# codyheiser/MILWRM

Measured on AMD Instinct MI355X. Metric: pixels/sec (node) for preprocess+k-means fit+label, 30-ch MxIF k=8; %HBM peak, higher is better.
Workload: dtype f32 (fp64 accumulation)

## Files before the change

include/milwrm_amd.h:

```cpp
#ifndef MILWRM_AMD_H
#define MILWRM_AMD_H

#include <stddef.h>
#include <stdint.h>

#ifdef __cplusplus
extern "C" {
#endif

#define MW_OK 0
#define MW_EINVAL (-1)
#define MW_EHIP (-2)
#define MW_EUNSUPPORTED (-3)

#define MW_U8 0
#define MW_U16 1
#define MW_F32 2

int mw_version(void);
const char* mw_last_error(void);
int mw_stream_blocks(int64_t n);
int64_t mw_rows_per_block(int64_t n);

size_t mw_nz_stats_ws_bytes(int64_t n_pix, int C);
// ... 234 lines not shown
  int64_t msg_len;
  int (*all_reduce_sum)(void* ctx, int64_t off, int64_t n, void* stream);
  int (*all_gather)(void* ctx, int64_t in_off, int64_t n, int64_t out_off, void* stream);
} mw_fit_comm;
int64_t mw_lloyd_fits_msg_len(int64_t rec_total, int F, int world);
int mw_lloyd_fits_sharded(const float* d_X, int64_t S, int F, const float* d_a32, const float* d_b32,
                          const int32_t* d_qexp, const float* h_a32, const float* h_b32,
                          const int32_t* h_qexp, const float* h_xmax, const double* h_mu,
                          const double* h_inv, int n, const int* h_k, const double* h_init,
                          uint8_t* const* d_labels, float* const* d_ub, float* const* d_lb,
                          void* const* d_ws, float* d_par, double* d_out, int max_iter, double tol,
                          int first_kind, int queue_kind, double queue_below, int dense_min,
                          int nobound, double* h_centers, double* h_inertia, int* h_n_iter,
                          int64_t* h_hist, int hist_cap, int* h_hist_len, double* h_timing,
                          const mw_fit_comm* comm, void* stream);

size_t mw_farthest_ws_bytes(int64_t S);
int mw_farthest(const float* d_X, int64_t S, int F, const float* d_a,
                const float* d_b, const double* d_centers, int k,
                const uint8_t* d_labels, int n, int64_t* d_top_idx,
                double* d_top_val, void* d_ws, void* stream);

size_t mw_assign_ws_bytes(int64_t n_pix, int k);
int mw_assign_conf(const float* d_img, int C, const int32_t* d_feat, int F,
                   const float* d_a, const float* d_b, const float* d_centers,
                   int k, const uint8_t* d_mask, int64_t n_pix,
                   int8_t* d_label, float* d_conf, void* d_ws, void* stream);
int mw_blur_assign_conf(const void* d_img, int dtype, int H, int W, int C, const float* d_inv_mean,
                        float pseudoval, const float* h_weights, int radius, const float* d_a,
                        const float* d_b, const float* d_centers, int k, const uint8_t* d_mask,
// ... 40 lines not shown
```

milwrm_amd/_native.py:

```python
from __future__ import annotations

import ctypes as C
import os
import threading

import torch

_HERE = os.path.dirname(os.path.abspath(__file__))
LIB_PATH = os.environ.get("MW_LIB") or os.path.join(_HERE, "libmilwrm_amd.so")

MW_U8, MW_U16, MW_F32 = 0, 1, 2
_EINVAL, _EHIP, _EUNSUP = -1, -2, -3

_lib = None
_lock = threading.Lock()

c_i64, c_i32, c_u32, c_u64 = C.c_int64, C.c_int, C.c_uint32, C.c_uint64
c_f32, c_sz, c_vp = C.c_float, C.c_size_t, C.c_void_p
c_dp = C.POINTER(C.c_double)

_PROTOS = {
    "mw_version": (c_i32, []),
    "mw_host_labels_f64": (c_i32, [c_vp, c_i64, c_vp, c_i32]),
    "mw_host_f32_to_f64": (c_i32, [c_vp, c_i64, c_vp, c_i32]),
# ... 75 lines not shown
                                            c_vp, c_vp]),
    "mw_kmeans_fit_deferred": (c_i32, [c_vp, c_i64, c_i32, c_vp, c_vp, c_vp, c_vp, c_i32, c_vp, c_u32, c_i32,
                                       C.c_double, c_vp, c_vp, c_vp, c_vp, c_vp, c_sz, c_i32, c_vp, c_vp, c_vp]),
    "mw_kmeans_fit_finish_ws_bytes": (c_sz, [c_i64, c_i32, c_i32]),
    "mw_kmeans_fit_finish": (c_i32, [c_vp, c_i64, c_i32, c_vp, c_vp, c_vp, c_i32, c_vp, c_i32, c_vp, c_vp, c_sz,
                                     c_vp, c_vp, c_vp]),
    "mw_lloyd_fits": (c_i32, [c_vp, c_i64, c_i32, c_vp, c_vp, c_vp, c_vp, c_vp, c_vp, c_vp, c_vp, c_vp,
                              c_i32, c_vp, c_vp, c_vp, c_vp, c_vp, c_vp, c_vp, c_vp, c_i32, C.c_double,
                              c_i32, c_i32, C.c_double, c_i32, c_i32, c_vp, c_vp, c_vp, c_vp, c_i32, c_vp,
                              c_vp, c_vp]),
    "mw_lloyd_fits_msg_len": (c_i64, [c_i64, c_i32, c_i32]),
    "mw_lloyd_fits_sharded": (c_i32, [c_vp, c_i64, c_i32, c_vp, c_vp, c_vp, c_vp, c_vp, c_vp, c_vp, c_vp, c_vp,
                                      c_i32, c_vp, c_vp, c_vp, c_vp, c_vp, c_vp, c_vp, c_vp, c_i32, C.c_double,
                                      c_i32, c_i32, C.c_double, c_i32, c_i32, c_vp, c_vp, c_vp, c_vp, c_i32,
                                      c_vp, c_vp, c_vp, c_vp]),
    "mw_farthest_ws_bytes": (c_sz, [c_i64]),
    "mw_farthest": (c_i32, [c_vp, c_i64, c_i32, c_vp, c_vp, c_vp, c_i32, c_vp, c_i32, c_vp, c_vp, c_vp, c_vp]),
    "mw_assign_ws_bytes": (c_sz, [c_i64, c_i32]),
    "mw_assign_conf": (c_i32, [c_vp, c_i32, c_vp, c_i32, c_vp, c_vp, c_vp, c_i32, c_vp, c_i64, c_vp, c_vp, c_vp, c_vp]),
    "mw_assign_reduce": (c_i32, [c_vp, c_i64, c_i32, c_vp, c_vp]),
    "mw_domain_sse_ws_bytes": (c_sz, [c_i64, c_i32, c_i32]),
    "mw_domain_sse_out_len": (c_i32, [c_i32, c_i32]),
    "mw_domain_sse": (c_i32, [c_vp, c_i32, c_vp, c_i32, c_vp, c_vp, c_vp, c_vp, c_vp, c_i32, c_i32, c_vp,
                              c_i64, c_vp, c_i32, c_vp, c_vp]),
    "mw_domain_sse_f64": (c_i32, [c_vp, c_i32, c_vp, c_i32, c_vp, c_vp, c_vp, c_vp, c_vp, c_i32, c_i32, c_vp,
                                  c_i64, c_vp, c_i32, c_vp, c_vp]),
    "mw_neighbor_mean": (c_i32, [c_vp, c_vp, c_i64, c_vp, c_i32, c_vp, c_vp]),
    "mw_col_stats_rows": (c_i32, [c_vp, c_i64, c_i32, c_vp, c_vp]),
    "mw_col_stats_absmax": (c_i32, [c_vp, c_i64, c_i32, c_vp, c_i32, c_vp]),
    "mw_sample_slot_elems": (c_sz, [c_i64]),
# ... 100 lines not shown
```

milwrm_amd/csrc/fit.cpp:

```cpp
#include <hip/hip_runtime.h>

#include <algorithm>
#include <chrono>
#include <cmath>
#include <cstring>
#include <limits>
#include <vector>

#include "common.h"

#pragma clang fp contract(off)

namespace mw {
void mt_init_genrand(uint32_t seed, uint32_t* mt);
void mt_regen(uint32_t* mt);
int kpp_step(const float* d_X, int64_t S, int F, const double* d_mu, const double* d_inv, int c,
             const double* h_u, int T, void* d_ws, void* stream, bool store_cur);

namespace {

struct LegacyRandom {
  uint32_t mt[624];
  int pos = 624;
  explicit LegacyRandom(uint32_t seed) { mt_init_genrand(seed, mt); }
// ... 285 lines not shown
    for (int i = 0; i < n; ++i)
      MW_HIP(hipMemcpyAsync(r.data() + (size_t)i * F, X + idx[i] * F, F * sizeof(float),
                            hipMemcpyDeviceToHost, st));
    MW_HIP(hipStreamSynchronize(st));
    for (int i = 0; i < n; ++i)
      for (int f = 0; f < F; ++f)
        outv[(size_t)i * F + f] = ((double)r[(size_t)i * F + f] - mu[f]) * inv[f];
    return MW_OK;
  }
};

struct FitLayout {
  size_t small, par, ub, lb, lws, out, big, fold, total;
};
static inline size_t fal(size_t x) { return (x + 255) & ~(size_t)255; }
static int lloyd_queue_kind() {
  static const int q = [] {
    const char* e = getenv("MW_LLOYD_LIST");
    return (e && e[0] == '0') ? 2 : 4;
  }();
  return q;
}
static FitLayout fit_layout(int64_t S, int F, int k) {
  const int T = 2 + (int)std::log((double)(k < 1 ? 1 : k));
  FitLayout L;
  L.small = 0;
  L.par = fal(64 * 4 * 4 + 64 * 8 * 2 + 64 * 64 * 8 + 64 * 8 * 2 + 130 * 8 + 64 * 8);
  L.ub = L.par + fal(((size_t)k * F + 2 * k) * 4);
  L.lb = L.ub + fal((size_t)S * 4);
  L.lws = L.lb + fal((size_t)S * 4);
// ... 348 lines not shown
      if (h_init_idx) std::memcpy(h_init_idx, idx.data(), k * sizeof(int64_t));
    } else {
      MW_HIP(hipMemcpyAsync(idx.data(), d_idx, k * 8, hipMemcpyDeviceToHost, st));
      MW_HIP(hipStreamSynchronize(st));
      idx[0] = first;
      MW_TRY(fit.scaled_rows(idx.data(), k, h_mu, h_inv, centers));
      if (h_init_idx) std::memcpy(h_init_idx, idx.data(), k * sizeof(int64_t));
    }
  }

  fit_hist.clear();
  if (!fold) MW_HIP(hipMemsetAsync(d_labels, 255, (size_t)S, st));
  std::vector<int64_t> q_hi((size_t)k * F, 0), q_lo((size_t)k * F, 0), count(k, 0);
  std::vector<double> rec, cnew((size_t)k * F), weight(k), tmp(std::max(F, k));
  int64_t last_recomputed = -1;
  int n_iter = 0;
  bool done = false, strict = false;
  for (int it = 0; it < max_iter && !done; ++it) {
    MW_TRY(fit.upload(centers));
    static const int first_kind = [] {
      const char* e = getenv("MW_LLOYD_FIRST_ATOMIC");
      return (e && e[0] == '1') ? 3 : 0;
    }();
    static const double queue_below = [] {
      const char* e = getenv("MW_LLOYD_QUEUE_BELOW");
      return e ? atof(e) : 0.3;
    }();
    const int queue_kind = lloyd_queue_kind();
    int kind = first_kind;
    if (last_recomputed >= 0) {
      double frac = (double)last_recomputed / (double)S;
      if (fit.prev_dmax > 0.f && std::isfinite(fit.drift_max))
        frac *= std::min(1.0, (double)fit.drift_max / (double)fit.prev_dmax);
      kind = frac > queue_below ? 1 : queue_kind;
    }
    if (fold && it == 0) {
      MW_TRY(mw_lloyd_list_moved(d_moved, mw_kpp_best_ptr(big, S, T), S, F, k, fit.ws, st));
      MW_TRY(fit.pass(0, 8, 0, rec, true));
    } else {
      MW_TRY(fit.pass(0, kind, 0, rec));
    }
    for (size_t i = 0; i < (size_t)k * F; ++i) {
      q_hi[i] += (int64_t)rec[i];
      q_lo[i] += (int64_t)rec[(size_t)k * F + i];
      const int64_t carry = q_lo[i] >> 32;
      q_hi[i] += carry;
      q_lo[i] -= carry << 32;
    }
    for (int j = 0; j < k; ++j) count[j] += (int64_t)rec[2 * (size_t)k * F + j];
    const double* tail = rec.data() + 2 * (size_t)k * F + k;
    const int64_t changed = (int64_t)tail[0];
    last_recomputed = (int64_t)tail[1];
    fit_hist.insert(fit_hist.end(), {(int64_t)(fold && it == 0 ? 8 : kind), changed, last_recomputed,
                                     (int64_t)(tail[2] * 4294967296.0 + tail[3])});
    for (int j = 0; j < k; ++j) {
      weight[j] = (double)count[j];
      for (int f = 0; f < F; ++f) {
        const size_t i = (size_t)j * F + f;
        const double sx = ((double)q_hi[i] * 4294967296.0 + (double)q_lo[i]) * qscale[f];
        cnew[i] = fit.a64[f] * sx + fit.b64[f] * weight[j];
      }
    }
    std::vector<int> empty;
    for (int j = 0; j < k; ++j)
      if (weight[j] == 0.0) empty.push_back(j);
    if (!empty.empty()) {
      const int ne = (int)empty.size();
// ... 57 lines not shown

  *h_n_iter = n_iter;
  std::memcpy(h_centers, centers.data(), centers.size() * sizeof(double));
  if (h_strict) {
    *h_strict = strict ? 1 : 0;
    return MW_OK;
  }
  fit_hist.insert(fit_hist.end(), {(int64_t)(strict ? 12 : 11), -1, -1, S});
  return fit_tail(fit, xmax.data(), centers, strict, !own.p, h_inertia, h_final_rec, h_inertia_exp);
}

namespace mw {
namespace {

constexpr int kFitsMaxPerLaunch = 24;
constexpr int kKindFirst = 0, kKindTile = 1, kKindDense = 5;

struct FitsFit {
  int k = 0;
  std::vector<double> centers;
  std::vector<float> prev32;
  bool have_prev = false;
  std::vector<int64_t> q_hi, q_lo, count;
  bool done = false, strict = false, bounds_ok = true;
  int n_iter = 0;
  double drift_max = 0.0, prev_dmax = 0.0;
  int iexp = 0;
  std::vector<int64_t> hist;
};

void fits_tables(FitsFit& fs, int F, bool nobound, float* h) {
  const int k = fs.k;
  for (size_t i = 0; i < (size_t)k * F; ++i) h[i] = (float)fs.centers[i];
  const float inf = std::numeric_limits<float>::infinity();
  std::vector<float> drift32(k), half32(k);
  double dmax;
  if (nobound) {
    for (int j = 0; j < k; ++j) drift32[j] = inf, half32[j] = 0.f;
    dmax = std::numeric_limits<double>::infinity();
  } else {
    std::vector<double> tmp(F);
// ... 62 lines not shown
  ~TimedLaunches() {
    for (T& t : v) {
      (void)hipEventDestroy(t.a);
      (void)hipEventDestroy(t.b);
    }
  }
};

int lloyd_fits_impl(const float* d_X, int64_t S, int F, const float* d_a32, const float* d_b32,
                    const int32_t* d_qexp, const float* h_a32, const float* h_b32, const int32_t* h_qexp,
                    const float* h_xmax, const double* h_mu, const double* h_inv, int n, const int* h_k,
                    const double* h_init, uint8_t* const* d_labels, float* const* d_ub, float* const* d_lb,
                    void* const* d_ws, float* d_par, double* d_out, int max_iter, double tol, int first_kind,
                    int queue_kind, double queue_below, int dense_min, int nobound, double* h_centers,
                    double* h_inertia, int* h_n_iter, int64_t* h_hist, int hist_cap, int* h_hist_len,
                    double* h_timing, const mw_fit_comm* comm, void* stream);

}
}

extern "C" int mw_lloyd_fits(const float* d_X, int64_t S, int F, const float* d_a32, const float* d_b32,
                             const int32_t* d_qexp, const float* h_a32, const float* h_b32,
                             const int32_t* h_qexp, const float* h_xmax, const double* h_mu,
                             const double* h_inv, int n, const int* h_k, const double* h_init,
                             uint8_t* const* d_labels, float* const* d_ub, float* const* d_lb,
                             void* const* d_ws, float* d_par, double* d_out, int max_iter, double tol,
                             int first_kind, int queue_kind, double queue_below, int dense_min,
                             int nobound, double* h_centers, double* h_inertia, int* h_n_iter,
                             int64_t* h_hist, int hist_cap, int* h_hist_len, double* h_timing,
                             void* stream) {
  return lloyd_fits_impl(d_X, S, F, d_a32, d_b32, d_qexp, h_a32, h_b32, h_qexp, h_xmax, h_mu, h_inv, n, h_k,
                         h_init, d_labels, d_ub, d_lb, d_ws, d_par, d_out, max_iter, tol, first_kind, queue_kind,
                         queue_below, dense_min, nobound, h_centers, h_inertia, h_n_iter, h_hist, hist_cap,
                         h_hist_len, h_timing, nullptr, stream);
}

extern "C" int64_t mw_lloyd_fits_msg_len(int64_t rec_total, int F, int world) {
  if (rec_total < 0 || F < 1 || F > 64 || world < 1) return 0;
  return msg_layout(rec_total, F, world).total;
}

extern "C" int mw_lloyd_fits_sharded(const float* d_X, int64_t S, int F, const float* d_a32,
                                     const float* d_b32, const int32_t* d_qexp, const float* h_a32,
                                     const float* h_b32, const int32_t* h_qexp, const float* h_xmax,
                                     const double* h_mu, const double* h_inv, int n, const int* h_k,
                                     const double* h_init, uint8_t* const* d_labels, float* const* d_ub,
                                     float* const* d_lb, void* const* d_ws, float* d_par, double* d_out,
                                     int max_iter, double tol, int first_kind, int queue_kind,
                                     double queue_below, int dense_min, int nobound, double* h_centers,
                                     double* h_inertia, int* h_n_iter, int64_t* h_hist, int hist_cap,
                                     int* h_hist_len, double* h_timing, const mw_fit_comm* comm,
                                     void* stream) {
  MW_CHECK_ARG(comm && comm->d_msg && comm->all_reduce_sum && comm->all_gather,
               "mw_lloyd_fits_sharded: null comm");
  MW_CHECK_ARG(comm->world >= 1 && comm->rank >= 0 && comm->rank < comm->world && comm->row_offset >= 0 &&
                   comm->rows_total >= S + comm->row_offset,
               "mw_lloyd_fits_sharded: bad world / rank / row range");
  MW_CHECK_ARG(d_out == comm->d_msg, "mw_lloyd_fits_sharded: d_out must be comm->d_msg (records at offset 0)");
  return lloyd_fits_impl(d_X, S, F, d_a32, d_b32, d_qexp, h_a32, h_b32, h_qexp, h_xmax, h_mu, h_inv, n, h_k,
                         h_init, d_labels, d_ub, d_lb, d_ws, d_par, d_out, max_iter, tol, first_kind, queue_kind,
                         queue_below, dense_min, nobound, h_centers, h_inertia, h_n_iter, h_hist, hist_cap,
                         h_hist_len, h_timing, comm, stream);
}

namespace mw {
namespace {

int lloyd_fits_impl(const float* d_X, int64_t S, int F, const float* d_a32, const float* d_b32,
                    const int32_t* d_qexp, const float* h_a32, const float* h_b32, const int32_t* h_qexp,
                    const float* h_xmax, const double* h_mu, const double* h_inv, int n, const int* h_k,
                    const double* h_init, uint8_t* const* d_labels, float* const* d_ub, float* const* d_lb,
                    void* const* d_ws, float* d_par, double* d_out, int max_iter, double tol, int first_kind,
                    int queue_kind, double queue_below, int dense_min, int nobound, double* h_centers,
                    double* h_inertia, int* h_n_iter, int64_t* h_hist, int hist_cap, int* h_hist_len,
                    double* h_timing, const mw_fit_comm* comm, void* stream) {
  MW_CHECK_ARG(d_X && d_a32 && d_b32 && d_qexp && h_a32 && h_b32 && h_qexp && h_xmax && h_mu && h_inv &&
                   h_k && h_init && d_labels && d_ub && d_lb && d_ws && d_par && d_out && h_centers &&
                   h_inertia && h_n_iter,
               "mw_lloyd_fits: null pointer");
  MW_CHECK_ARG(n >= 1 && F >= 1 && F <= 64 && S >= 1 && max_iter >= 1 && tol >= 0.0,
               "mw_lloyd_fits: bad n / F / S / max_iter / tol");
  hipStream_t st = as_stream(stream);
  const int64_t S_glob = comm ? comm->rows_total : S;
  std::vector<FitsFit> fits(n);
  std::vector<int64_t> poff(n + 1, 0), roff(n + 1, 0);
  size_t coff = 0;
  for (int g = 0; g < n; ++g) {
    const int k = h_k[g];
    MW_CHECK_ARG(k >= 1 && k <= 64 && S >= k, "mw_lloyd_fits: fit %d: k=%d", g, k);
    FitsFit& fs = fits[g];
    fs.k = k;
    fs.centers.assign(h_init + coff, h_init + coff + (size_t)k * F);
    coff += (size_t)k * F;
    fs.q_hi.assign((size_t)k * F, 0);
    fs.q_lo.assign((size_t)k * F, 0);
    fs.count.assign(k, 0);
// ... 125 lines not shown
  double* d_c64 = nullptr;
  int64_t* d_topi = nullptr;
  double* d_topv = nullptr;
  void* d_farws = nullptr;

  int rc = MW_OK;
  std::vector<double> cnew, weight, tmp(std::max(F, kmax));
  for (int it = 0; it < max_iter && rc == MW_OK; ++it) {
    std::vector<int> active;
    for (int g = 0; g < n; ++g)
      if (!fits[g].done) active.push_back(g);
    if (active.empty()) break;
    const bool dense_now = dense_ok && it > 0 && (int)active.size() >= dense_min;
    if ((rc = upload(active)) != MW_OK) break;
    std::vector<int> by_kind[8];
    for (int g : active) {
      const FitsFit& fs = fits[g];
      int kind;
      if (fs.hist.empty()) {
        kind = first_kind;
      } else if (dense_now) {
        kind = kKindDense;
      } else if (!fs.bounds_ok) {
        kind = kKindTile;
      } else {
        double frac = (double)fs.hist.back() / (double)std::max<int64_t>(S_glob, 1);
        if (fs.prev_dmax > 0 && std::isfinite(fs.drift_max)) frac *= std::min(1.0, fs.drift_max / fs.prev_dmax);
        kind = frac > queue_below ? kKindTile : queue_kind;
      }
      by_kind[kind].push_back(g);
    }
    host_mark();
    for (int kind = 0; kind < 8 && rc == MW_OK; ++kind)
      if (!by_kind[kind].empty()) rc = launch(by_kind[kind], 0, kind);
    if (rc != MW_OK || (rc = download()) != MW_OK) break;
    for (int g : active) {
      FitsFit& fs = fits[g];
      const int k = fs.k;
      if (it > 0) fs.bounds_ok = !dense_now;
      const double* r = rec + roff[g];
      for (size_t i = 0; i < (size_t)k * F; ++i) {
        fs.q_hi[i] += (int64_t)r[i];
        fs.q_lo[i] += (int64_t)r[(size_t)k * F + i];
        const int64_t carry = fs.q_lo[i] >> 32;
        fs.q_hi[i] += carry;
        fs.q_lo[i] -= carry << 32;
      }
      for (int j = 0; j < k; ++j) fs.count[j] += (int64_t)r[2 * (size_t)k * F + j];
      const double* tail = r + 2 * (size_t)k * F + k;
      const int64_t changed = (int64_t)tail[0];
      fs.hist.push_back(changed);
      fs.hist.push_back((int64_t)tail[1]);
      cnew.assign((size_t)k * F, 0.0);
      weight.assign(k, 0.0);
      for (int j = 0; j < k; ++j) {
        weight[j] = (double)fs.count[j];
        for (int f = 0; f < F; ++f) {
          const size_t i = (size_t)j * F + f;
          const double sx = ((double)fs.q_hi[i] * 4294967296.0 + (double)fs.q_lo[i]) * qscale[f];
          cnew[i] = a64[f] * sx + b64[f] * weight[j];
        }
      }
      std::vector<int> empty;
      for (int j = 0; j < k; ++j)
        if (weight[j] == 0.0) empty.push_back(j);
      if (!empty.empty()) {
        const int ne = (int)empty.size();
// ... 198 lines not shown
```

milwrm_amd/csrc/lloyd.hip:

```cpp
#include <math.h>
#include <stdlib.h>

#include "kmeans_common.h"

namespace mw {
constexpr int kLloydBlocksF32 = 3 * 256;
static inline int lloyd_blocks(int64_t S, int F) {
  const int g = kblocks(S);
  return (F <= 32 && g > kLloydBlocksF32) ? kLloydBlocksF32 : g;
}
static inline int64_t lloyd_rows(int64_t S, int F) {
  int64_t tiles = (S + kT - 1) / kT;
  if (tiles < 1) tiles = 1;
  const int g = lloyd_blocks(S, F);
  return ((tiles + g - 1) / g) * kT;
}
}

namespace mw {

constexpr int kMaxFits = 24;
constexpr float kEps = 1e-4f;

struct LloydFitsArg {
// ... 35 lines not shown
};

__host__ __device__ inline size_t lloyd_lds_bytes(int FMAX, int k, int F, int mode, int kind) {
  size_t b = sizeof(LloydSmall) + cent_t_bytes(64, FMAX);
  if (mode == 0) b += ((size_t)k * F * 8 + 15) & ~(size_t)15;
  b += 4 * (lloyd_tile_bytes(FMAX, F) + 64 * 4);
  if (mode == 0 && kind == 2) b += (size_t)kChunk * 2;
  return b;
}

constexpr int kFirst = 0;
constexpr int kTile = 1;
constexpr int kQueue = 2;
constexpr int kFirstAtomic = 3;
constexpr int kList = 4;
constexpr int kFirstSum = 7;
constexpr int kListGiven = 8;

template <int FMAX, int MODE, int KIND, int MBT>
__device__ __forceinline__ void lloyd_pass_body(const float* __restrict__ X, int64_t S, int F,
                                                const float* __restrict__ ga, const float* __restrict__ gb,
                                                const int* __restrict__ qexp, const LloydFitsArg& fits, int n,
                                                int64_t R) {
  constexpr int NV = FMAX / 4;
  constexpr int RP = 64 / FMAX;
  constexpr int NB = FMAX <= 16 ? 1 : FMAX / 16;
  extern __shared__ __attribute__((aligned(16))) char smem[];
  const int g = blockIdx.x % n, blk = blockIdx.x / n;
  const mw_lloyd_fit& fit = fits.f[g];
  const int k = fit.k;
// ... 386 lines not shown
        continue;
      } else {
        f2v x2[FMAX / 2];
        load_scaled_row<FMAX>(s_tile, lane, F, s_a, s_b, x2);
        if (MODE == 2) {
          const float d = dist_one<FMAX>(x2, s_cT, lab_old < k ? lab_old : 0);
          if (valid) inert += fixq(d, iexp);
          continue;
        }
        int lab;
        float m1, m2;
        nearest_centers<FMAX, 64, true>(x2, s_cT, k, lab, m1, m2);
        recomputed += valid ? 1 : 0;
        const bool ch = valid && lab != lab_old;
        changed += ch ? 1 : 0;
        if (valid) __builtin_amdgcn_raw_buffer_store_b8((unsigned char)lab, rl, lane, tc * 64, 0);
        if (MODE == 1) {
          if (valid) inert += fixq(m1, iexp);
          continue;
        }
        if (valid) {
          __builtin_amdgcn_raw_buffer_store_b32(__builtin_bit_cast(int, sqrtf(m1)), ru, lane * 4, tc * 256, 0);
          __builtin_amdgcn_raw_buffer_store_b32(
              __builtin_bit_cast(int, k > 1 ? sqrtf(m2) : __builtin_inff()), rw, lane * 4, tc * 256, 0);
        }
        if constexpr (MODE == 0 && KIND == kFirstAtomic) {
          move_rows(__ballot(ch), lab, 255);
          continue;
        }
        if constexpr (MODE == 0 && KIND == kFirstSum) {
          const float* xcol = s_tile + (lane < F ? lane : 0);
#pragma unroll
          for (int j = 0; j < KS; ++j) {
            if (j >= k) break;
            unsigned long long m = __ballot(valid && lab == j);
            if (lane == 0 && m) atomicAdd(&s_cnt[j], __popcll(m));
            double sj = 0.0;
            while (m != 0ull) {
              int r[4];
#pragma unroll
              for (int u = 0; u < 4; ++u) {
                r[u] = m != 0ull ? __builtin_ctzll(m) : -1;
// ... 313 lines not shown
               "mw_lloyd_list_moved: bad arguments");
  const int G = lloyd_blocks(S, F);
  hipLaunchKernelGGL(lloyd_list_moved_kernel, dim3(G), dim3(256), 0, as_stream(stream), d_moved, d_best, S,
                     lloyd_rows(S, F), static_cast<char*>(d_ws), lloyd_list_off(G, k, F), G);
  MW_LAUNCH_CHECK();
  return MW_OK;
}

int mw_lloyd_pass(const float* d_X, int64_t S, int F, const float* d_a, const float* d_b,
                  const int32_t* d_qexp, int n, const mw_lloyd_fit* h_fits, int mode, int kind,
                  void* stream) {
  MW_CHECK_ARG(d_X && d_a && d_b && d_qexp && h_fits, "mw_lloyd_pass: null pointer");
  MW_CHECK_ARG(S > 0 && F > 0 && n >= 1 && n <= kMaxFits, "mw_lloyd_pass: bad shape (1 <= n <= %d)",
               kMaxFits);
  MW_CHECK_ARG(mode >= 0 && mode <= 2, "mw_lloyd_pass: bad mode %d", mode);
  MW_CHECK_ARG(kind >= 0 && kind <= 6 || kind == kListGiven, "mw_lloyd_pass: bad kind %d", kind);
  const bool lists_given = kind == kListGiven;
  if (lists_given) {
    MW_CHECK_ARG(mode == 0 && S < ((int64_t)1 << 31), "mw_lloyd_pass: kind 8 needs mode 0 and S < 2^31");
    kind = kList;
  }
  if (mode != 0) kind = kFirst;
  if (kind == kList && S >= ((int64_t)1 << 31)) kind = kQueue;
  LloydFitsArg fits{};
  int kmax = 0;
  for (int g = 0; g < n; ++g) {
    const mw_lloyd_fit& f = h_fits[g];
    MW_CHECK_ARG(f.centers && f.labels && f.ws && f.out && f.k >= 1, "mw_lloyd_pass: fit %d: bad arguments", g);
    MW_CHECK_ARG(mode != 0 || (f.ub && f.lb && f.drift && f.half_sep),
                 "mw_lloyd_pass: fit %d: mode 0 needs ub, lb, drift, half_sep", g);
    fits.f[g] = f;
    kmax = f.k > kmax ? f.k : kmax;
  }
  if (kmax > 64 || F > 64) {
    set_error("mw_lloyd_pass: k=%d F=%d unsupported (k <= 64, F <= 64)", kmax, F);
    return MW_EUNSUPPORTED;
  }
  hipStream_t s = as_stream(stream);
  const int G = lloyd_blocks(S, F);
  const int64_t R = lloyd_rows(S, F);
  if (kind == kDense || kind == kDense + 1) {
    DenseArg da{};
    if (!dense_groups(h_fits, n, da)) {
      set_error("mw_lloyd_pass: dense kind needs k <= %d per fit", kDenseMaxFitK);
      return MW_EUNSUPPORTED;
    }
    MW_CHECK_ARG(kind == kDense || [&] {
      for (int g = 0; g < n; ++g)
        if (!h_fits[g].ub || !h_fits[g].lb) return false;
      return true;
    }(), "mw_lloyd_pass: kind 6 needs ub / lb");
    da.bounds = kind == kDense ? 0 : (int)((1u << n) - 1u);
    static const float bscale = [] {
      const char* e = getenv("MW_DENSE_BSCALE");
      const float v = e ? (float)atof(e) : kDenseBScale;
      return v > kDenseBScale ? v : kDenseBScale;
    }();
    da.bscale = bscale;
    da.G = G;
    static const bool use2 = [] {
      const char* e = getenv("MW_DENSE2");
      return !(e && e[0] == '0');
    }();
    Dense2Arg d2{};
    if (use2 && dense2_plan(h_fits, n, S, F, d2)) {
      d2.bounds = da.bounds;
// ... 44 lines not shown
  if (mode == 0 && kind == kList && !lists_given) {
    hipLaunchKernelGGL(lloyd_mark_kernel, grid, dim3(256), 0, s, fits, n, S, F, R);
    MW_LAUNCH_CHECK();
  }
#define MW_LP(FMV, MO, KI, MBV)                                                                        \
  hipLaunchKernelGGL((lloyd_pass_kernel<FMV, MO, KI, MBV>), grid, dim3(256), lds, s, d_X, S, F, d_a, d_b, \
                     d_qexp, fits, n, R)
#define MW_LPF(FMV)                                                              \
  if (mode == 0) {                                                               \
    if (kind == kFirst) {                                                        \
      if (MBF == 1) MW_LP(FMV, 0, kFirst, 1);                                    \
      else if (MBF == 2) { if constexpr ((FMV <= 32)) MW_LP(FMV, 0, kFirst, 2); } \
      else { if constexpr ((FMV <= 16)) MW_LP(FMV, 0, kFirst, 4); }              \
    }                                                                            \
    else if (kind == kTile) MW_LP(FMV, 0, kTile, 1);                            \
    else if (kind == kFirstAtomic) MW_LP(FMV, 0, kFirstAtomic, 1);              \
    else if (kind == kFirstSum) MW_LP(FMV, 0, kFirstSum, 1);                    \
    else if (kind == kList) MW_LP(FMV, 0, kList, 1);                            \
    else MW_LP(FMV, 0, kQueue, 1);                                              \
  } else if (mode == 1) MW_LP(FMV, 1, kFirst, 1);                               \
  else MW_LP(FMV, 2, kFirst, 1);
  static const bool first_w2 = [] {
    const char* e = getenv("MW_LLOYD_FIRST_W2");
    return !(e && e[0] == '0');
  }();
  if (first_w2 && FM == 64 && mode == 0 && (kind == kFirst || kind == kFirstSum) && MBF == 1) {
    if (kind == kFirst)
      hipLaunchKernelGGL((lloyd_first_w2_kernel<64, kFirst>), grid, dim3(256), lds, s, d_X, S, F, d_a, d_b, d_qexp,
                         fits, n, R);
    else
// ... 27 lines not shown
```

milwrm_amd/csrc/lloyd_dense.h:

```cpp
#pragma once

namespace mw {

constexpr int kDense = 5;
constexpr int kDenseMaxK = 64;
constexpr int kDenseMaxFits = 8;
constexpr int kDenseSD = 68;
constexpr int kDenseMaxFitK = 20;

struct DenseGroup {
  int g0, n;
  int off[kDenseMaxFits + 1];
};
struct DenseArg {
  DenseGroup grp[kMaxFits];
  int ngroups;
  int G;
  int bounds;
  float bscale;
};

typedef _Float16 h8d __attribute__((ext_vector_type(8)));
typedef float f4d __attribute__((ext_vector_type(4)));

// ... 317 lines not shown
```

milwrm_amd/kmeans.py:

```python
from __future__ import annotations

import ctypes as C
import os
import warnings

import numpy as np
import torch

from . import _native as N
from . import device as D
from . import profiling
from .rng import as_random_state, first_center_index, kpp_draws


class DeviceRows:

    def __init__(self, X: torch.Tensor, mu=None, inv=None, feature_var=None, xmax_local=None):
        assert X.dtype == torch.float32 and X.dim() == 2 and X.is_contiguous()
        self.X = X
        self.S, self.F = X.shape
        self.mu = np.zeros(self.F) if mu is None else np.asarray(mu, dtype=np.float64)
        self.inv = np.ones(self.F) if inv is None else np.asarray(inv, dtype=np.float64)
        self.a_host = self.inv.astype(np.float32)
        self.b_host = (-self.mu * self.inv).astype(np.float32)
        self._dev_affine = None
        self._feature_var = feature_var
        self.xmax = None
        self._xmax_local = None if xmax_local is None else np.asarray(xmax_local, np.float32)
        self.qexp_dev = None
        self.draws = None
        self.moments = None

    def moment_segments(self):
        m = self.moments
        if not m or len(m) > 16 or sum(n for _, n, _, _ in m) != self.S:
            return None
        arr = (N.KppSeg * len(m))()
        for i, (off, n, rpb, rec) in enumerate(m):
            arr[i] = N.KppSeg(int(off), int(n), int(rpb), D.P(rec))
        return len(m), arr

    def spatial_order(self):
        if not self.draws or sum(S for _, S, _, _ in self.draws) != self.S:
            return None
        keys = torch.empty(self.S, dtype=torch.int64, device=self.X.device)
        for off, S, idx, base in self.draws:
# ... 264 lines not shown
        self.q_lo = np.zeros((k, F), dtype=np.int64)
        self.count = np.zeros(k, dtype=np.int64)
        self.labels = torch.full((S,), 255, dtype=torch.uint8, device=dev)
        self.ub = torch.empty(S, dtype=torch.float32, device=dev)
        self.lb = torch.empty(S, dtype=torch.float32, device=dev)
        self.ws = torch.empty(lloyd_ws_bytes(S, k, F), dtype=torch.uint8, device=dev)
        self.done = False
        self.strict = False
        self.n_iter = 0
        self.recomputed = 0
        self.history = []
        self.iexp = 0
        self.drift_max = 0.0
        self.prev_dmax = 0.0
        self.bounds_ok = True

    def add(self, rec, F, qscale, a64, b64):
        k = self.k
        hi = rec[:k * F].reshape(k, F).astype(np.int64)
        lo = rec[k * F:2 * k * F].reshape(k, F).astype(np.int64)
        self.q_hi += hi
        self.q_lo += lo
        carry = self.q_lo >> 32
        self.q_hi += carry
        self.q_lo -= carry << 32
        self.count += rec[2 * k * F:2 * k * F + k].astype(np.int64)
        tail = rec[2 * k * F + k:]
        self.recomputed += int(tail[1])
        self.history.append((int(tail[0]), int(tail[1])))
        sums_x = (self.q_hi.astype(np.float64) * 4294967296.0 + self.q_lo.astype(np.float64)) * qscale
        cnt = self.count.astype(np.float64)
        return a64[None, :] * sums_x + b64[None, :] * cnt[:, None], cnt, tail[0]


KIND_FIRST, KIND_TILE, KIND_QUEUE, KIND_LIST, KIND_DENSE = 0, 1, 2, 4, 5
DENSE_MIN_FITS = int(os.environ.get("MW_LLOYD_DENSE_MIN", "3"))
SWEEP_SORT = os.environ.get("MW_SWEEP_SORT", "1") != "0"
DENSE_MODE = os.environ.get("MW_LLOYD_DENSE", "auto")
USE_DENSE = DENSE_MODE != "0"
QUEUE_KIND = KIND_QUEUE if os.environ.get("MW_LLOYD_LIST") == "0" else KIND_LIST


def lloyd_ws_bytes(S: int, k: int, F: int) -> int:
    return N.query("mw_lloyd_ws_bytes_kinds", S, k, F, int(QUEUE_KIND == KIND_LIST))
QUEUE_BELOW = float(os.environ.get("MW_LLOYD_QUEUE_BELOW", "0.3"))
USE_C_FIT = os.environ.get("MW_KMEANS_C", "1") != "0"


def _launch_pass(rows, fits_g, mode, kind, par, poff, outs, st, label="lloyd_pass"):
    S, F = rows.S, rows.F
    arr = (N.LloydFit * len(fits_g))()
    nbytes = 0
    for i, (g, fs) in enumerate(fits_g):
        base = D.P(par) + int(poff[g]) * 4
        k = fs.k
        arr[i] = N.LloydFit(base, base + k * F * 4, base + (k * F + k) * 4, D.P(fs.labels),
                            D.P(fs.ub), D.P(fs.lb), D.P(fs.ws), D.P(outs[g]), k,
                            float(fs.drift_max), int(fs.iexp))
        if kind == KIND_DENSE:
            nbytes += 2 * S + (S * F * 4 if i == 0 else 0)
        else:
            nbytes += S * 9 + (S * F * 4 if (mode or kind not in (KIND_QUEUE, KIND_LIST)) else 0)
    tag = "" if mode else ("_first", "_tile", "_queue", "_first_atomic", "_list", "_dense", "_dense")[kind]
    ev = None
    if TRACE is not None:
        ev = (torch.cuda.Event(enable_timing=True), torch.cuda.Event(enable_timing=True))
        ev[0].record()
    with profiling.timed(f"{label}_mode{mode}{tag}", nbytes):
        N.call("mw_lloyd_pass", D.P(rows.X), S, F, D.P(rows.a32), D.P(rows.b32), D.P(rows.qexp_dev),
               len(fits_g), C.addressof(arr), int(mode), int(kind), st)
    if ev is not None:
        ev[1].record()
        TRACE.append({"mode": mode, "kind": tag.strip("_"), "fits": [g for g, _ in fits_g], "ev": ev})


TRACE = [] if os.environ.get("MW_LLOYD_TRACE") == "1" else None


# ... 56 lines not shown

    def run(sel, mode, kind_of):
        by_kind = {}
        for g in sel:
            by_kind.setdefault(kind_of(g), []).append(g)
        for kind, gs in sorted(by_kind.items()):
            for i in range(0, len(gs), 24):
                _launch_pass(rows, [(g, fits[g]) for g in gs[i:i + 24]], mode, kind, par, poff,
                             outs, st)
        comm.all_reduce_(out_all)
        return D.d2h(out_all)

    first = 3 if os.environ.get("MW_LLOYD_FIRST_ATOMIC") == "1" else KIND_FIRST

    dense_now = [False]

    def kind_of(g):
        fs = fits[g]
        if not fs.history:
            return first
        if dense_now[0]:
            return KIND_DENSE
        if not fs.bounds_ok:
            return KIND_TILE
        frac = fs.history[-1][1] / max(S_glob, 1)
        if fs.prev_dmax > 0 and np.isfinite(fs.drift_max):
            frac *= min(1.0, fs.drift_max / fs.prev_dmax)
        return KIND_TILE if frac > QUEUE_BELOW else QUEUE_KIND

    dense_ok = USE_DENSE and F <= (64 if DENSE_MODE == "1" else 30) and max(ks) <= 20
    if use_c:
        hook = None
        if sizes is not None:
            hook = _CommHook(comm, msg, S_glob, int(sizes[:comm.rank].sum()))
        return _lloyd_fits_c(rows, fits, rls, out_all, par, max_iter, tol, dense_ok, first, st, hook)
    for it in range(max_iter):
        active = [g for g in range(n) if not fits[g].done]
        if not active:
            break
        dense_now[0] = dense_ok and it > 0 and len(active) >= DENSE_MIN_FITS
        upload(active)
        rec_all = run(active, 0, kind_of)
        for g in active:
            fs = fits[g]
            if it > 0:
                fs.bounds_ok = not dense_now[0]
            sums, weight, changed = fs.add(rec_all[roff[g]:roff[g + 1]], F, qscale, a64, b64)
            centers_new = sums.copy()
            _relocate_empty(rows, fs.labels, fs.centers, centers_new, weight, comm)
            _average_centers(centers_new, weight)
            shift = np.sqrt(((centers_new - fs.centers) ** 2).sum(axis=1))
            fs.centers = centers_new
            fs.n_iter = it + 1
            if verbose:
                print(f"Iteration {it}: {int(changed)} labels changed.")
            if changed == 0:
                fs.strict = fs.done = True
                if verbose:
                    print(f"Converged at iteration {it}: strict convergence.")
            elif (shift ** 2).sum() <= tol:
                fs.done = True
                if verbose:
# ... 17 lines not shown
    rec_all = D.d2h(out_all)
    res = []
    for g, fs in enumerate(fits):
        tail = rec_all[roff[g + 1] - 4:roff[g + 1]]
        inertia = float((tail[2] * 4294967296.0 + tail[3]) * 2.0 ** -fs.iexp)
        res.append((fs.labels, inertia, fs.centers, fs.n_iter))
    LAST_STATS["recomputed"] = [fs.recomputed for fs in fits]
    LAST_STATS["history"] = [fs.history for fs in fits]
    return res


LAST_STATS = {}
USE_C_FITS = os.environ.get("MW_LLOYD_FITS_C", "1") != "0"
_PASS_NAMES = ["lloyd_pass_mode0_first", "lloyd_pass_mode0_tile", "lloyd_pass_mode0_queue",
               "lloyd_pass_mode0_first_atomic", "lloyd_pass_mode0_list", "lloyd_pass_mode0_dense",
               "lloyd_pass_mode0_dense", "lloyd_pass_mode1", "lloyd_pass_mode2"]


FITS_C_USED = {"local": 0, "sharded": 0}


class _CommHook:

    def __init__(self, comm, msg: torch.Tensor, rows_total: int, row_offset: int):
        self.comm, self.msg, self.err = comm, msg, None
        self._ar = N.ALL_REDUCE_SUM_FN(self._all_reduce)
        self._ag = N.ALL_GATHER_FN(self._all_gather)
        self.struct = N.FitComm(None, comm.world, comm.rank, int(rows_total), int(row_offset), D.P(msg),
                                msg.numel(), self._ar, self._ag)
        self.reduces = 0

# ... 5 lines not shown
        except BaseException as e:
            self.err = e
            return 1

    def _all_gather(self, ctx, in_off, n, out_off, stream):
        try:
            g = self.comm.all_gather_t(self.msg[in_off:in_off + n])
            self.msg[out_off:out_off + self.comm.world * n].copy_(
                torch.from_numpy(np.ascontiguousarray(g, dtype=np.float64).reshape(-1)))
            return 0
        except BaseException as e:
            self.err = e
            return 1


def _lloyd_fits_c(rows, fits, rls, out_all, par, max_iter, tol, dense_ok, first, st, hook=None):
    S, F = rows.S, rows.F
    n = len(fits)
    ptrs = lambda ts: (C.c_void_p * n)(*[D.P(t) for t in ts])
    h_k = np.array([fs.k for fs in fits], dtype=np.int32)
    h_init = np.ascontiguousarray(np.concatenate([fs.centers.ravel() for fs in fits]), dtype=np.float64)
    centers = np.empty_like(h_init)
    inertia = np.empty(n, dtype=np.float64)
    n_iter = np.empty(n, dtype=np.int32)
    hist = np.zeros((n, max_iter, 2), dtype=np.int64)
    hist_len = np.zeros(n, dtype=np.int32)
    timing = np.zeros(30, dtype=np.float64) if profiling.enabled() else None
    a32 = np.ascontiguousarray(rows.a_host, dtype=np.float32)
    b32 = np.ascontiguousarray(rows.b_host, dtype=np.float32)
    qexp = np.ascontiguousarray(rows.qexp, dtype=np.int32)
    xmax = np.ascontiguousarray(rows.xmax, dtype=np.float32)
    mu = np.ascontiguousarray(rows.mu, dtype=np.float64)
    inv = np.ascontiguousarray(rows.inv, dtype=np.float64)
    nobound = int(os.environ.get("MW_LLOYD_NOBOUND") == "1")
    args = (D.P(rows.X), S, F, D.P(rows.a32), D.P(rows.b32), D.P(rows.qexp_dev),
            a32.ctypes.data, b32.ctypes.data, qexp.ctypes.data, xmax.ctypes.data, mu.ctypes.data,
            inv.ctypes.data, n, h_k.ctypes.data, h_init.ctypes.data,
            ptrs([fs.labels for fs in fits]), ptrs([fs.ub for fs in fits]), ptrs([fs.lb for fs in fits]),
            ptrs([fs.ws for fs in fits]), D.P(par), D.P(out_all), int(max_iter), float(tol), int(first),
            int(QUEUE_KIND), float(QUEUE_BELOW), int(DENSE_MIN_FITS) if dense_ok else -1, nobound,
            centers.ctypes.data, inertia.ctypes.data, n_iter.ctypes.data, hist.ctypes.data, int(max_iter),
            hist_len.ctypes.data, None if timing is None else timing.ctypes.data)
    if hook is None:
        N.call("mw_lloyd_fits", *args, st)
        FITS_C_USED["local"] += 1
    else:
        status = N.load().mw_lloyd_fits_sharded(*args, C.byref(hook.struct), st)
        if hook.err is not None:
            raise hook.err
        N.check(status, "mw_lloyd_fits_sharded")
        FITS_C_USED["sharded"] += 1
    if timing is not None:
        for slot, name in enumerate(_PASS_NAMES):
            profiling.add_measured(name, int(timing[3 * slot]), timing[3 * slot + 1], timing[3 * slot + 2])
        profiling.add_measured("lloyd_fits_host", int(timing[27]), timing[28], 0)
        if hook is not None:
            profiling.add_measured("lloyd_fits_comm", int(timing[27]), timing[29], 0)
    res = []
    o = 0
    for g, fs in enumerate(fits):
        kF = fs.k * F
        fs.centers = centers[o:o + kF].reshape(fs.k, F).copy()
# ... 60 lines not shown
            inits[i], km.init_indices_ = km._kpp(rows, as_random_state(km.random_state), comm)
    tols = {km._tol for km in models}
    max_iters = {km.max_iter for km in models}
    assert len(tols) == 1 and len(max_iters) == 1
    perm = None
    if SWEEP_SORT and len(models) > 1 and rows.draws:
        from .stream import RESIDENCY
        need = fit_memory_need(rows, [km.n_clusters for km in models]) + sort_memory_need(rows)
        if RESIDENCY.release(need) >= need:
            perm = rows.spatial_order()
    lrows = rows
    if perm is not None:
        lrows = DeviceRows(rows.X.index_select(0, perm), rows.mu, rows.inv, feature_var=rows._feature_var,
                           xmax_local=rows._xmax_local)
        lrows.xmax, lrows.qexp_dev = rows.xmax, rows.qexp_dev
        if rows.qexp_dev is not None:
            lrows.qexp = rows.qexp
    res = lloyd_fits(lrows, inits, max_iters.pop(), tols.pop(), False, comm)
    del lrows
    for km, (labels, inertia, centers, n_iter) in zip(models, res):
        if perm is not None:
            back = torch.empty_like(labels)
            back[perm] = labels
            labels = back
        km._set_fitted(rows, labels, inertia, centers, n_iter)
    return models


class _Inertia:

# ... 250 lines not shown
```

Before: 6.547 billion.

## Add full-streamed Lloyd kind that writes and moves only changed labels

Adds a new Lloyd pass kind (kFull) that streams every row but stores labels and updates center sums only for rows whose label changed, moving each changed row from its old cluster to its new one. The intent is to cut label write traffic and atomic sum updates in the late iterations, when few rows move. The queue-switching heuristic now uses a carried 'share' estimate rather than the last recomputed count, and the old tile kind is kept for spatially sorted sweep rows. This changes when the cheaper queue kind is chosen and depends on the incremental sums staying exactly consistent.

```diff
diff --git a/include/milwrm_amd.h b/include/milwrm_amd.h
--- a/include/milwrm_amd.h
+++ b/include/milwrm_amd.h
@@ -272,6 +272,16 @@
                           int nobound, double* h_centers, double* h_inertia, int* h_n_iter,
                           int64_t* h_hist, int hist_cap, int* h_hist_len, double* h_timing,
                           const mw_fit_comm* comm, void* stream);
+int mw_lloyd_fits_streamed(const float* d_X, int64_t S, int F, const float* d_a32, const float* d_b32,
+                           const int32_t* d_qexp, const float* h_a32, const float* h_b32,
+                           const int32_t* h_qexp, const float* h_xmax, const double* h_mu,
+                           const double* h_inv, int n, const int* h_k, const double* h_init,
+                           uint8_t* const* d_labels, float* const* d_ub, float* const* d_lb,
+                           void* const* d_ws, float* d_par, double* d_out, int max_iter, double tol,
+                           int first_kind, int queue_kind, double queue_below, int dense_min,
+                           int nobound, double* h_centers, double* h_inertia, int* h_n_iter,
+                           int64_t* h_hist, int hist_cap, int* h_hist_len, double* h_timing,
+                           const mw_fit_comm* comm, int streamed_kind, void* stream);
 
 size_t mw_farthest_ws_bytes(int64_t S);
 int mw_farthest(const float* d_X, int64_t S, int F, const float* d_a,
diff --git a/milwrm_amd/_native.py b/milwrm_amd/_native.py
--- a/milwrm_amd/_native.py
+++ b/milwrm_amd/_native.py
@@ -113,6 +113,10 @@
                                       c_i32, c_vp, c_vp, c_vp, c_vp, c_vp, c_vp, c_vp, c_vp, c_i32, C.c_double,
                                       c_i32, c_i32, C.c_double, c_i32, c_i32, c_vp, c_vp, c_vp, c_vp, c_i32,
                                       c_vp, c_vp, c_vp, c_vp]),
+    "mw_lloyd_fits_streamed": (c_i32, [c_vp, c_i64, c_i32, c_vp, c_vp, c_vp, c_vp, c_vp, c_vp, c_vp, c_vp, c_vp,
+                                       c_i32, c_vp, c_vp, c_vp, c_vp, c_vp, c_vp, c_vp, c_vp, c_i32, C.c_double,
+                                       c_i32, c_i32, C.c_double, c_i32, c_i32, c_vp, c_vp, c_vp, c_vp, c_i32,
+                                       c_vp, c_vp, c_vp, c_i32, c_vp]),
     "mw_farthest_ws_bytes": (c_sz, [c_i64]),
     "mw_farthest": (c_i32, [c_vp, c_i64, c_i32, c_vp, c_vp, c_vp, c_i32, c_vp, c_i32, c_vp, c_vp, c_vp, c_vp]),
     "mw_assign_ws_bytes": (c_sz, [c_i64, c_i32]),
diff --git a/milwrm_amd/csrc/fit.cpp b/milwrm_amd/csrc/fit.cpp
--- a/milwrm_amd/csrc/fit.cpp
+++ b/milwrm_amd/csrc/fit.cpp
@@ -323,6 +323,7 @@
   size_t small, par, ub, lb, lws, out, big, fold, total;
 };
 static inline size_t fal(size_t x) { return (x + 255) & ~(size_t)255; }
+constexpr int kKindFirst = 0, kKindTile = 1, kKindDense = 5, kKindFull = 6;
 static int lloyd_queue_kind() {
   static const int q = [] {
     const char* e = getenv("MW_LLOYD_LIST");
@@ -701,6 +702,7 @@
   std::vector<int64_t> q_hi((size_t)k * F, 0), q_lo((size_t)k * F, 0), count(k, 0);
   std::vector<double> rec, cnew((size_t)k * F), weight(k), tmp(std::max(F, k));
   int64_t last_recomputed = -1;
+  double share = 1.0;
   int n_iter = 0;
   bool done = false, strict = false;
   for (int it = 0; it < max_iter && !done; ++it) {
@@ -715,11 +717,12 @@
     }();
     const int queue_kind = lloyd_queue_kind();
     int kind = first_kind;
+    double frac = 1.0;
     if (last_recomputed >= 0) {
-      double frac = (double)last_recomputed / (double)S;
+      frac = share;
       if (fit.prev_dmax > 0.f && std::isfinite(fit.drift_max))
         frac *= std::min(1.0, (double)fit.drift_max / (double)fit.prev_dmax);
-      kind = frac > queue_below ? 1 : queue_kind;
+      kind = frac > queue_below ? kKindFull : queue_kind;
     }
     if (fold && it == 0) {
       MW_TRY(mw_lloyd_list_moved(d_moved, mw_kpp_best_ptr(big, S, T), S, F, k, fit.ws, st));
@@ -738,6 +741,7 @@
     const double* tail = rec.data() + 2 * (size_t)k * F + k;
     const int64_t changed = (int64_t)tail[0];
     last_recomputed = (int64_t)tail[1];
+    share = kind == kKindFull ? std::min(1.0, frac) : (double)last_recomputed / (double)S;
     fit_hist.insert(fit_hist.end(), {(int64_t)(fold && it == 0 ? 8 : kind), changed, last_recomputed,
                                      (int64_t)(tail[2] * 4294967296.0 + tail[3])});
     for (int j = 0; j < k; ++j) {
@@ -825,7 +829,6 @@
 namespace {
 
 constexpr int kFitsMaxPerLaunch = 24;
-constexpr int kKindFirst = 0, kKindTile = 1, kKindDense = 5;
 
 struct FitsFit {
   int k = 0;
@@ -836,6 +839,7 @@
   bool done = false, strict = false, bounds_ok = true;
   int n_iter = 0;
   double drift_max = 0.0, prev_dmax = 0.0;
+  double share = 1.0;
   int iexp = 0;
   std::vector<int64_t> hist;
 };
@@ -928,7 +932,7 @@
                     void* const* d_ws, float* d_par, double* d_out, int max_iter, double tol, int first_kind,
                     int queue_kind, double queue_below, int dense_min, int nobound, double* h_centers,
                     double* h_inertia, int* h_n_iter, int64_t* h_hist, int hist_cap, int* h_hist_len,
-                    double* h_timing, const mw_fit_comm* comm, void* stream);
+                    double* h_timing, const mw_fit_comm* comm, int streamed_kind, void* stream);
 
 }
 }
@@ -946,7 +950,7 @@
   return lloyd_fits_impl(d_X, S, F, d_a32, d_b32, d_qexp, h_a32, h_b32, h_qexp, h_xmax, h_mu, h_inv, n, h_k,
                          h_init, d_labels, d_ub, d_lb, d_ws, d_par, d_out, max_iter, tol, first_kind, queue_kind,
                          queue_below, dense_min, nobound, h_centers, h_inertia, h_n_iter, h_hist, hist_cap,
-                         h_hist_len, h_timing, nullptr, stream);
+                         h_hist_len, h_timing, nullptr, kKindFull, stream);
 }
 
 extern "C" int64_t mw_lloyd_fits_msg_len(int64_t rec_total, int F, int world) {
@@ -965,16 +969,35 @@
                                      double* h_inertia, int* h_n_iter, int64_t* h_hist, int hist_cap,
                                      int* h_hist_len, double* h_timing, const mw_fit_comm* comm,
                                      void* stream) {
-  MW_CHECK_ARG(comm && comm->d_msg && comm->all_reduce_sum && comm->all_gather,
-               "mw_lloyd_fits_sharded: null comm");
-  MW_CHECK_ARG(comm->world >= 1 && comm->rank >= 0 && comm->rank < comm->world && comm->row_offset >= 0 &&
-                   comm->rows_total >= S + comm->row_offset,
-               "mw_lloyd_fits_sharded: bad world / rank / row range");
-  MW_CHECK_ARG(d_out == comm->d_msg, "mw_lloyd_fits_sharded: d_out must be comm->d_msg (records at offset 0)");
+  MW_CHECK_ARG(comm, "mw_lloyd_fits_sharded: null comm");
+  return mw_lloyd_fits_streamed(d_X, S, F, d_a32, d_b32, d_qexp, h_a32, h_b32, h_qexp, h_xmax, h_mu, h_inv, n, h_k,
+                                h_init, d_labels, d_ub, d_lb, d_ws, d_par, d_out, max_iter, tol, first_kind,
+                                queue_kind, queue_below, dense_min, nobound, h_centers, h_inertia, h_n_iter,
+                                h_hist, hist_cap, h_hist_len, h_timing, comm, kKindFull, stream);
+}
+
+extern "C" int mw_lloyd_fits_streamed(const float* d_X, int64_t S, int F, const float* d_a32,
+                                      const float* d_b32, const int32_t* d_qexp, const float* h_a32,
+                                      const float* h_b32, const int32_t* h_qexp, const float* h_xmax,
+                                      const double* h_mu, const double* h_inv, int n, const int* h_k,
+                                      const double* h_init, uint8_t* const* d_labels, float* const* d_ub,
+                                      float* const* d_lb, void* const* d_ws, float* d_par, double* d_out,
+                                      int max_iter, double tol, int first_kind, int queue_kind,
+                                      double queue_below, int dense_min, int nobound, double* h_centers,
+                                      double* h_inertia, int* h_n_iter, int64_t* h_hist, int hist_cap,
+                                      int* h_hist_len, double* h_timing, const mw_fit_comm* comm,
+                                      int streamed_kind, void* stream) {
+  if (comm) {
+    MW_CHECK_ARG(comm->d_msg && comm->all_reduce_sum && comm->all_gather, "mw_lloyd_fits_sharded: null comm");
+    MW_CHECK_ARG(comm->world >= 1 && comm->rank >= 0 && comm->rank < comm->world && comm->row_offset >= 0 &&
+                     comm->rows_total >= S + comm->row_offset,
+                 "mw_lloyd_fits_sharded: bad world / rank / row range");
+    MW_CHECK_ARG(d_out == comm->d_msg, "mw_lloyd_fits_sharded: d_out must be comm->d_msg (records at offset 0)");
+  }
   return lloyd_fits_impl(d_X, S, F, d_a32, d_b32, d_qexp, h_a32, h_b32, h_qexp, h_xmax, h_mu, h_inv, n, h_k,
                          h_init, d_labels, d_ub, d_lb, d_ws, d_par, d_out, max_iter, tol, first_kind, queue_kind,
                          queue_below, dense_min, nobound, h_centers, h_inertia, h_n_iter, h_hist, hist_cap,
-                         h_hist_len, h_timing, comm, stream);
+                         h_hist_len, h_timing, comm, streamed_kind, stream);
 }
 
 namespace mw {
@@ -987,13 +1010,15 @@
                     void* const* d_ws, float* d_par, double* d_out, int max_iter, double tol, int first_kind,
                     int queue_kind, double queue_below, int dense_min, int nobound, double* h_centers,
                     double* h_inertia, int* h_n_iter, int64_t* h_hist, int hist_cap, int* h_hist_len,
-                    double* h_timing, const mw_fit_comm* comm, void* stream) {
+                    double* h_timing, const mw_fit_comm* comm, int streamed_kind, void* stream) {
   MW_CHECK_ARG(d_X && d_a32 && d_b32 && d_qexp && h_a32 && h_b32 && h_qexp && h_xmax && h_mu && h_inv &&
                    h_k && h_init && d_labels && d_ub && d_lb && d_ws && d_par && d_out && h_centers &&
                    h_inertia && h_n_iter,
                "mw_lloyd_fits: null pointer");
   MW_CHECK_ARG(n >= 1 && F >= 1 && F <= 64 && S >= 1 && max_iter >= 1 && tol >= 0.0,
                "mw_lloyd_fits: bad n / F / S / max_iter / tol");
+  MW_CHECK_ARG(streamed_kind == kKindTile || streamed_kind == kKindFull, "mw_lloyd_fits: streamed_kind %d (1 or 6)",
+               streamed_kind);
   hipStream_t st = as_stream(stream);
   const int64_t S_glob = comm ? comm->rows_total : S;
   std::vector<FitsFit> fits(n);
@@ -1149,6 +1174,8 @@
     const bool dense_now = dense_ok && it > 0 && (int)active.size() >= dense_min;
     if ((rc = upload(active)) != MW_OK) break;
     std::vector<int> by_kind[8];
+    std::vector<int> kind_g(n, 0);
+    std::vector<double> frac_g(n, 1.0);
     for (int g : active) {
       const FitsFit& fs = fits[g];
       int kind;
@@ -1159,10 +1186,12 @@
       } else if (!fs.bounds_ok) {
         kind = kKindTile;
       } else {
-        double frac = (double)fs.hist.back() / (double)std::max<int64_t>(S_glob, 1);
+        double frac = fs.share;
         if (fs.prev_dmax > 0 && std::isfinite(fs.drift_max)) frac *= std::min(1.0, fs.drift_max / fs.prev_dmax);
-        kind = frac > queue_below ? kKindTile : queue_kind;
-      }
+        kind = frac > queue_below ? streamed_kind : queue_kind;
+        frac_g[g] = frac;
+      }
+      kind_g[g] = kind;
       by_kind[kind].push_back(g);
     }
     host_mark();
@@ -1186,6 +1215,8 @@
       const int64_t changed = (int64_t)tail[0];
       fs.hist.push_back(changed);
       fs.hist.push_back((int64_t)tail[1]);
+      fs.share = kind_g[g] == kKindFull ? std::min(1.0, frac_g[g])
+                                        : (double)fs.hist.back() / (double)std::max<int64_t>(S_glob, 1);
       cnew.assign((size_t)k * F, 0.0);
       weight.assign(k, 0.0);
       for (int j = 0; j < k; ++j) {
diff --git a/milwrm_amd/csrc/lloyd.hip b/milwrm_amd/csrc/lloyd.hip
--- a/milwrm_amd/csrc/lloyd.hip
+++ b/milwrm_amd/csrc/lloyd.hip
@@ -73,6 +73,7 @@
 constexpr int kQueue = 2;
 constexpr int kFirstAtomic = 3;
 constexpr int kList = 4;
+constexpr int kFull = 6;
 constexpr int kFirstSum = 7;
 constexpr int kListGiven = 8;
 
@@ -489,7 +490,8 @@
         recomputed += valid ? 1 : 0;
         const bool ch = valid && lab != lab_old;
         changed += ch ? 1 : 0;
-        if (valid) __builtin_amdgcn_raw_buffer_store_b8((unsigned char)lab, rl, lane, tc * 64, 0);
+        if (MODE == 0 && KIND == kFull ? ch : valid)
+          __builtin_amdgcn_raw_buffer_store_b8((unsigned char)lab, rl, lane, tc * 64, 0);
         if (MODE == 1) {
           if (valid) inert += fixq(m1, iexp);
           continue;
@@ -501,6 +503,10 @@
         }
         if constexpr (MODE == 0 && KIND == kFirstAtomic) {
           move_rows(__ballot(ch), lab, 255);
+          continue;
+        }
+        if constexpr (MODE == 0 && KIND == kFull) {
+          move_rows(__ballot(ch), lab, lab_old);
           continue;
         }
         if constexpr (MODE == 0 && KIND == kFirstSum) {
@@ -844,7 +850,8 @@
   MW_CHECK_ARG(S > 0 && F > 0 && n >= 1 && n <= kMaxFits, "mw_lloyd_pass: bad shape (1 <= n <= %d)",
                kMaxFits);
   MW_CHECK_ARG(mode >= 0 && mode <= 2, "mw_lloyd_pass: bad mode %d", mode);
-  MW_CHECK_ARG(kind >= 0 && kind <= 6 || kind == kListGiven, "mw_lloyd_pass: bad kind %d", kind);
+  MW_CHECK_ARG(kind >= 0 && kind <= 6 || kind == kListGiven || kind == kDenseBounds, "mw_lloyd_pass: bad kind %d",
+               kind);
   const bool lists_given = kind == kListGiven;
   if (lists_given) {
     MW_CHECK_ARG(mode == 0 && S < ((int64_t)1 << 31), "mw_lloyd_pass: kind 8 needs mode 0 and S < 2^31");
@@ -869,7 +876,7 @@
   hipStream_t s = as_stream(stream);
   const int G = lloyd_blocks(S, F);
   const int64_t R = lloyd_rows(S, F);
-  if (kind == kDense || kind == kDense + 1) {
+  if (kind == kDense || kind == kDenseBounds) {
     DenseArg da{};
     if (!dense_groups(h_fits, n, da)) {
       set_error("mw_lloyd_pass: dense kind needs k <= %d per fit", kDenseMaxFitK);
@@ -879,7 +886,7 @@
       for (int g = 0; g < n; ++g)
         if (!h_fits[g].ub || !h_fits[g].lb) return false;
       return true;
-    }(), "mw_lloyd_pass: kind 6 needs ub / lb");
+    }(), "mw_lloyd_pass: kind 9 needs ub / lb");
     da.bounds = kind == kDense ? 0 : (int)((1u << n) - 1u);
     static const float bscale = [] {
       const char* e = getenv("MW_DENSE_BSCALE");
@@ -954,6 +961,7 @@
       else { if constexpr ((FMV <= 16)) MW_LP(FMV, 0, kFirst, 4); }              \
     }                                                                            \
     else if (kind == kTile) MW_LP(FMV, 0, kTile, 1);                            \
+    else if (kind == kFull) MW_LP(FMV, 0, kFull, 1);                            \
     else if (kind == kFirstAtomic) MW_LP(FMV, 0, kFirstAtomic, 1);              \
     else if (kind == kFirstSum) MW_LP(FMV, 0, kFirstSum, 1);                    \
     else if (kind == kList) MW_LP(FMV, 0, kList, 1);                            \
diff --git a/milwrm_amd/csrc/lloyd_dense.h b/milwrm_amd/csrc/lloyd_dense.h
--- a/milwrm_amd/csrc/lloyd_dense.h
+++ b/milwrm_amd/csrc/lloyd_dense.h
@@ -3,6 +3,7 @@
 namespace mw {
 
 constexpr int kDense = 5;
+constexpr int kDenseBounds = 9;
 constexpr int kDenseMaxK = 64;
 constexpr int kDenseMaxFits = 8;
 constexpr int kDenseSD = 68;
diff --git a/milwrm_amd/kmeans.py b/milwrm_amd/kmeans.py
--- a/milwrm_amd/kmeans.py
+++ b/milwrm_amd/kmeans.py
@@ -30,6 +30,7 @@
         self.qexp_dev = None
         self.draws = None
         self.moments = None
+        self.slide_order = False
 
     def moment_segments(self):
         m = self.moments
@@ -324,6 +325,7 @@
         self.drift_max = 0.0
         self.prev_dmax = 0.0
         self.bounds_ok = True
+        self.share = 1.0
 
     def add(self, rec, F, qscale, a64, b64):
         k = self.k
@@ -343,7 +345,8 @@
         return a64[None, :] * sums_x + b64[None, :] * cnt[:, None], cnt, tail[0]
 
 
-KIND_FIRST, KIND_TILE, KIND_QUEUE, KIND_LIST, KIND_DENSE = 0, 1, 2, 4, 5
+KIND_FIRST, KIND_TILE, KIND_QUEUE, KIND_LIST, KIND_DENSE, KIND_FULL = 0, 1, 2, 4, 5, 6
+STREAMED_KIND = KIND_FULL
 DENSE_MIN_FITS = int(os.environ.get("MW_LLOYD_DENSE_MIN", "3"))
 SWEEP_SORT = os.environ.get("MW_SWEEP_SORT", "1") != "0"
 DENSE_MODE = os.environ.get("MW_LLOYD_DENSE", "auto")
@@ -371,7 +374,7 @@
             nbytes += 2 * S + (S * F * 4 if i == 0 else 0)
         else:
             nbytes += S * 9 + (S * F * 4 if (mode or kind not in (KIND_QUEUE, KIND_LIST)) else 0)
-    tag = "" if mode else ("_first", "_tile", "_queue", "_first_atomic", "_list", "_dense", "_dense")[kind]
+    tag = "" if mode else ("_first", "_tile", "_queue", "_first_atomic", "_list", "_dense", "_full")[kind]
     ev = None
     if TRACE is not None:
         ev = (torch.cuda.Event(enable_timing=True), torch.cuda.Event(enable_timing=True))
@@ -458,26 +461,32 @@
     first = 3 if os.environ.get("MW_LLOYD_FIRST_ATOMIC") == "1" else KIND_FIRST
 
     dense_now = [False]
+    streamed = KIND_TILE if rows.slide_order else STREAMED_KIND
+    picked = {}
 
     def kind_of(g):
         fs = fits[g]
+        frac = 1.0
         if not fs.history:
-            return first
-        if dense_now[0]:
-            return KIND_DENSE
-        if not fs.bounds_ok:
-            return KIND_TILE
-        frac = fs.history[-1][1] / max(S_glob, 1)
-        if fs.prev_dmax > 0 and np.isfinite(fs.drift_max):
-            frac *= min(1.0, fs.drift_max / fs.prev_dmax)
-        return KIND_TILE if frac > QUEUE_BELOW else QUEUE_KIND
+            kind = first
+        elif dense_now[0]:
+            kind = KIND_DENSE
+        elif not fs.bounds_ok:
+            kind = KIND_TILE
+        else:
+            frac = fs.share
+            if fs.prev_dmax > 0 and np.isfinite(fs.drift_max):
+                frac *= min(1.0, fs.drift_max / fs.prev_dmax)
+            kind = streamed if frac > QUEUE_BELOW else QUEUE_KIND
+        picked[g] = (kind, frac)
+        return kind
 
     dense_ok = USE_DENSE and F <= (64 if DENSE_MODE == "1" else 30) and max(ks) <= 20
     if use_c:
         hook = None
         if sizes is not None:
             hook = _CommHook(comm, msg, S_glob, int(sizes[:comm.rank].sum()))
-        return _lloyd_fits_c(rows, fits, rls, out_all, par, max_iter, tol, dense_ok, first, st, hook)
+        return _lloyd_fits_c(rows, fits, rls, out_all, par, max_iter, tol, dense_ok, first, st, hook, streamed)
     for it in range(max_iter):
         active = [g for g in range(n) if not fits[g].done]
         if not active:
@@ -490,6 +499,8 @@
             if it > 0:
                 fs.bounds_ok = not dense_now[0]
             sums, weight, changed = fs.add(rec_all[roff[g]:roff[g + 1]], F, qscale, a64, b64)
+            kind, frac = picked[g]
+            fs.share = min(1.0, frac) if kind == KIND_FULL else fs.history[-1][1] / max(S_glob, 1)
             centers_new = sums.copy()
             _relocate_empty(rows, fs.labels, fs.centers, centers_new, weight, comm)
             _average_centers(centers_new, weight)
@@ -537,7 +548,7 @@
 USE_C_FITS = os.environ.get("MW_LLOYD_FITS_C", "1") != "0"
 _PASS_NAMES = ["lloyd_pass_mode0_first", "lloyd_pass_mode0_tile", "lloyd_pass_mode0_queue",
                "lloyd_pass_mode0_first_atomic", "lloyd_pass_mode0_list", "lloyd_pass_mode0_dense",
-               "lloyd_pass_mode0_dense", "lloyd_pass_mode1", "lloyd_pass_mode2"]
+               "lloyd_pass_mode0_full", "lloyd_pass_mode1", "lloyd_pass_mode2"]
 
 
 FITS_C_USED = {"local": 0, "sharded": 0}
@@ -573,7 +584,8 @@
             return 1
 
 
-def _lloyd_fits_c(rows, fits, rls, out_all, par, max_iter, tol, dense_ok, first, st, hook=None):
+def _lloyd_fits_c(rows, fits, rls, out_all, par, max_iter, tol, dense_ok, first, st, hook=None,
+                  streamed=KIND_FULL):
     S, F = rows.S, rows.F
     n = len(fits)
     ptrs = lambda ts: (C.c_void_p * n)(*[D.P(t) for t in ts])
@@ -601,10 +613,10 @@
             centers.ctypes.data, inertia.ctypes.data, n_iter.ctypes.data, hist.ctypes.data, int(max_iter),
             hist_len.ctypes.data, None if timing is None else timing.ctypes.data)
     if hook is None:
-        N.call("mw_lloyd_fits", *args, st)
+        N.call("mw_lloyd_fits_streamed", *args, None, int(streamed), st)
         FITS_C_USED["local"] += 1
     else:
-        status = N.load().mw_lloyd_fits_sharded(*args, C.byref(hook.struct), st)
+        status = N.load().mw_lloyd_fits_streamed(*args, C.byref(hook.struct), int(streamed), st)
         if hook.err is not None:
             raise hook.err
         N.check(status, "mw_lloyd_fits_sharded")
@@ -695,6 +707,7 @@
         lrows = DeviceRows(rows.X.index_select(0, perm), rows.mu, rows.inv, feature_var=rows._feature_var,
                            xmax_local=rows._xmax_local)
         lrows.xmax, lrows.qexp_dev = rows.xmax, rows.qexp_dev
+        lrows.slide_order = True
         if rows.qexp_dev is not None:
             lrows.qexp = rows.qexp
     res = lloyd_fits(lrows, inits, max_iters.pop(), tols.pop(), False, comm)
```

Result: no change. 6.674 billion, median of 4 (+1.9%).
